# yahoo/bftkv

Measured on AMD Instinct MI355X. Metric: pgp_rsa2048_signature_verifies_per_sec, higher is better.
Workload: dtype u32; 1 GPU; 64-replica quorum, 10000 RSA-2048 signed writes per GPU (cfg2 of BASELINE.json), 534164 signature packets per GPU, 1.0% corrupt / 0.5% unknown issuer / 0.5% duplicate / 1.0% one-short; parallelism=shard-by-write x1, RCCL all-gather of verdict bitmaps on the verifier's stream, replicas=64, writes_per_gpu=10000, sigs_per_gpu=534164, batches_in_flight=3

## Files before the change

bftkv_amd/csrc/capi.hip:

```cpp
#include "../../include/bftkv_gpu.h"

#include <hip/hip_runtime.h>
#include <stdio.h>
#include <stdlib.h>
#include <string.h>

#include <limits.h>
#include <linux/futex.h>
#include <sched.h>
#include <sys/syscall.h>
#include <unistd.h>

#include <algorithm>
#include <array>
#include <atomic>
#include <memory>
#include <functional>
#include <map>
#include <set>
#include <chrono>
#include <condition_variable>
#include <mutex>
#include <shared_mutex>
#include <system_error>
// ... 33 lines not shown
  hipError_t ensure_exact(size_t bytes) {
    if (bytes <= cap) return hipSuccess;
    if (p) { hipError_t e = hipFree(p); if (e != hipSuccess) return e; p = nullptr; cap = 0; }
    hipError_t e = hipMalloc(&p, bytes);
    if (e == hipSuccess) cap = bytes;
    return e;
  }
  void release() { if (p) (void)hipFree(p); p = nullptr; cap = 0; }
  template <typename T> T* as() const { return (T*)p; }
};

struct KeyEntry {
  uint64_t key_id = 0, entity_id = 0;
  uint8_t algo = 0, flags = 0;
  uint32_t bits = 0, e = 0, n0 = 0, qbits = 0, n0_29 = 0;
  std::vector<uint32_t> nl29, r2_29;
  std::vector<uint32_t> nl, r2, r2w, qw, dtab, qpow, qconst;
  std::string material;
  bool cert_only = false;
  int cert_group = -1;
  uint32_t entity_index = 0;
  std::string cert_digest;
  uint64_t last_used = 0;
  bool dsa_unslotted = false;
};

struct QuorumHost {
  bool live = false;
  int n_qcs = 0;
  int32_t f[MAX_QC], mn[MAX_QC], thr[MAX_QC], suff[MAX_QC];
// ... 520 lines not shown
                           c->hash_mask.as<uint32_t>(), c->mid.as<uint32_t>(), c->mid64.as<uint64_t>());
        hipLaunchKernelGGL(k_hash_mid_text, dim3((n_items + 63) / 64, N_HASHES), dim3(64), 0, sh, d_tbs, d_tbs_off, n_items, c->hash_mask.as<uint32_t>(), txt);
      }
      hipLaunchKernelGGL(k_digest_sha256, dim3((total + 255) / 256), dim3(256), 0, sh, d_tbs, d_tbs_off, d_ss,
                         d_mid_in ? d_mid_in : c->mid.as<uint32_t>(), c->mid64.as<uint64_t>(), n_items, c->recs.as<SigRec>(), total,
                         c->digests.as<uint32_t>(), d_tbs_prefix, n_recs_dev);
    }
    HIPCHK(c, rec(6, sh));
    return 0;
  };
  if (!upload_tbs) { int hrc = hash_stream_work(); if (hrc) return hrc; }
  const dim3 qg((total + MODEXP_BLOCK / MONT_TPI - 1) / (MODEXP_BLOCK / MONT_TPI));
  const dim3 qg8((total + MODEXP_BLOCK / MONT_TPI_BIG - 1) / (MODEXP_BLOCK / MONT_TPI_BIG));
  static const bool wide8_off = getenv("BFTKV_NO_WIDE8") != nullptr;
  const bool wide8 = staged_cap != 0 && ss_len / 256 <= 8192 && !wide8_off;
  auto launch_modexp = [&](const uint32_t* start) {
    if (wide8)
      hipLaunchKernelGGL((k_rsa_modexp<10, MONT_TPI_BIG>), qg8, dim3(MODEXP_BLOCK), 0, s, d_ss, c->recs.as<SigRec>(), c->pk_list.as<uint32_t>(),
                         cnt_p, start, c->kt, c->r.as<uint32_t>(), c->xr.as<uint32_t>(), (uint64_t*)(cnt_p + 16));
    else {
#if BFTKV_RSA_FORM == 29
      hipLaunchKernelGGL((k_rsa_modexp<RSA29_L, MONT_TPI, RSA29_W>), qg, dim3(MODEXP_BLOCK), c->modexp_lds_pad, s, d_ss, c->recs.as<SigRec>(), c->pk_list.as<uint32_t>(),
                         cnt_p, start, c->kt, c->r.as<uint32_t>(), c->xr.as<uint32_t>(), (uint64_t*)(cnt_p + 16), (const uint32_t*)(cnt_p + 5));
      hipLaunchKernelGGL((k_rsa_modexp<MONT_L, MONT_TPI, MONT_W, true>), qg, dim3(MODEXP_BLOCK), c->modexp_lds_pad, s, d_ss, c->recs.as<SigRec>(), c->pk_list.as<uint32_t>(),
                         cnt_p, start, c->kt, c->r.as<uint32_t>(), c->xr.as<uint32_t>(), (uint64_t*)nullptr, (const uint32_t*)(cnt_p + 5));
#else
      hipLaunchKernelGGL((k_rsa_modexp<MONT_L, MONT_TPI>), qg, dim3(MODEXP_BLOCK), c->modexp_lds_pad, s, d_ss, c->recs.as<SigRec>(), c->pk_list.as<uint32_t>(),
                         cnt_p, start, c->kt, c->r.as<uint32_t>(), c->xr.as<uint32_t>(), (uint64_t*)(cnt_p + 16));
#endif
    }
    if (c->have_rsa3072)
      hipLaunchKernelGGL((k_rsa_modexp<MONT_L3072, MONT_TPI_BIG>), qg8, dim3(MODEXP_BLOCK), 0, s, d_ss, c->recs.as<SigRec>(), c->pk_list3072.as<uint32_t>(),
                         cnt_p + 2, start + 2, c->kt, c->r3072.as<uint32_t>(), c->xr.as<uint32_t>(), (uint64_t*)nullptr);
    if (c->have_rsa4096)
      hipLaunchKernelGGL((k_rsa_modexp<MONT_L4096, MONT_TPI_BIG>), qg8, dim3(MODEXP_BLOCK), 0, s, d_ss, c->recs.as<SigRec>(), c->pk_list4096.as<uint32_t>(),
                         cnt_p + 3, start + 3, c->kt, c->r4096.as<uint32_t>(), c->xr.as<uint32_t>(), (uint64_t*)nullptr);
  };
  static const bool turnstile_off = getenv("BFTKV_NO_TURNSTILE") != nullptr;
  const bool big = staged_cap ? (ev_input != nullptr && ss_len / 320 >= TURNSTILE_MIN_PACKETS) : total >= TURNSTILE_MIN_PACKETS;
  if (big && !turnstile_off) {
    Turnstile& g = g_turnstile[(unsigned)c->device & 15u];
    std::lock_guard<std::mutex> tl(g.mu);
    if (g.last && g.owner != c) HIPCHK(c, hipStreamWaitEvent(s, g.last, 0));
    HIPCHK(c, rec(9, s));
    launch_modexp(start0);
    if (!c->ev_turn) HIPCHK(c, hipEventCreateWithFlags(&c->ev_turn, hipEventDisableTiming));
    HIPCHK(c, hipEventRecord(c->ev_turn, s));
    g.last = c->ev_turn; g.owner = c;
  } else {
    HIPCHK(c, rec(9, s));
    if (total) launch_modexp(start0);
// ... 13 lines not shown
    for (uint32_t it = 0;; ++it) {
      const uint32_t v = __atomic_load_n(&c->h_mail[3], __ATOMIC_ACQUIRE);
      if (v) { other_hashes = (v & 1u) != 0; break; }
      if ((it & 255u) == 255u && std::chrono::steady_clock::now() - t_spin > std::chrono::microseconds(300) + std::chrono::nanoseconds((uint64_t)total / 2)) break;
      __builtin_ia32_pause();
    }
  }
  if (total && !d_mid_in && other_hashes)
    hipLaunchKernelGGL(k_digest_other, dim3(std::min<uint32_t>((total + 255) / 256, DIGEST_OTHER_MAX_BLOCKS)), dim3(256), 0, s,
                       d_tbs, d_tbs_off, d_ss, c->mid.as<uint32_t>(), c->mid64.as<uint64_t>(), n_items, c->recs.as<SigRec>(), total,
                       c->digests.as<uint32_t>(), c->pk_count.as<uint32_t>() + 4, txt, n_recs_dev);
  const dim3 cg(((uint64_t)total * CMP_LANES + 255) / 256);
  auto launch_compare = [&](const uint32_t* start) {
    hipLaunchKernelGGL(k_rsa_compare, cg, dim3(256), 0, s, c->recs.as<SigRec>(), c->pk_list.as<uint32_t>(),
                       cnt_p, start, c->kt, c->r.as<uint32_t>(), c->digests.as<uint32_t>());
    if (c->have_rsa3072)
      hipLaunchKernelGGL(k_rsa_compare, cg, dim3(256), 0, s, c->recs.as<SigRec>(), c->pk_list3072.as<uint32_t>(),
                         cnt_p + 2, start + 2, c->kt, c->r3072.as<uint32_t>(), c->digests.as<uint32_t>());
    if (c->have_rsa4096)
      hipLaunchKernelGGL(k_rsa_compare, cg, dim3(256), 0, s, c->recs.as<SigRec>(), c->pk_list4096.as<uint32_t>(),
                         cnt_p + 3, start + 3, c->kt, c->r4096.as<uint32_t>(), c->digests.as<uint32_t>());
  };
  auto launch_dsa = [&](const uint32_t* start) {
    hipLaunchKernelGGL(k_dsa_mul, dim3((total + 63) / 64), dim3(64), 0, s, c->recs.as<SigRec>(), c->dsa_list.as<uint32_t>(),
                       cnt_p, start, c->kt, c->digests.as<uint32_t>(), c->dsa_u.as<uint32_t>());
    const uint32_t* idx_s = nullptr; const uint32_t* idx_b = nullptr; const uint32_t* cnt_cls = nullptr;
    if (c->have_dsa3072 && c->have_dsa2048) {
      uint32_t* cc = cnt_p + (start == start0 ? 20 : 22);
      uint32_t* is = c->dsa_idx.as<uint32_t>() + (start == start0 ? 0 : 2 * (size_t)total);
      hipLaunchKernelGGL(k_dsa_split, dim3((total + 255) / 256), dim3(256), 0, s, c->recs.as<SigRec>(), c->dsa_list.as<uint32_t>(), cnt_p, start, c->kt,
// ... 44 lines not shown
  e.material.push_back((char)k.usable_sign);
  auto app = [&](const uint8_t* p, uint32_t l) {
    uint32_t z = 0;
    while (z < l && p[z] == 0) ++z;
    if (l > z) e.material.append((const char*)p + z, l - z);
    e.material.push_back('|');
  };
  app(k.n, k.n_len); app(k.e, k.e_len); app(k.g, k.g_len); app(k.y, k.y_len);
  e.flags = 0;
  if (k.usable_sign) e.flags |= KEYF_USABLE_SIGN;
  if (k.pk_algo != PK_RSA_ENCRYPT_ONLY && k.pk_algo != PK_ELGAMAL) e.flags |= KEYF_CAN_SIGN;
  if (k.key_id == k.entity_id) e.flags |= KEYF_PRIMARY;
  if (cert_only) e.flags |= KEYF_CERT_ONLY;
  e.bits = (uint32_t)hostbn::bit_length(k.n, k.n_len);
  e.e = 0; e.n0 = 0; e.qbits = 0;
  e.r2w.clear(); e.nl29.clear(); e.r2_29.clear(); e.n0_29 = 0;
  e.nl.assign(MONT_NMAX, 0); e.r2.assign(MONT_NMAX, 0); e.qw.assign(8, 0); e.dtab.assign(2 * DSA_N_BIG, 0); e.qpow.clear(); e.qconst.clear();
  if (k.pk_algo == PK_RSA || k.pk_algo == PK_RSA_SIGN_ONLY) {
    if (hostbn::bit_length(k.e, k.e_len) > 32) return fail(c, BFTKV_E_UNSUPPORTED, "RSA public exponent wider than 32 bits");
    for (uint32_t j = 0; j < k.e_len; ++j) e.e = (e.e << 8) | k.e[j];
    const int nlimbs = e.bits <= 2048 ? MONT_N : (e.bits <= 3072 ? MONT_TPI_BIG * MONT_L3072 : MONT_TPI_BIG * MONT_L4096);
    if (e.bits > 4096) e.bits = 0xFFFFFFFFu;
    else if (!hostbn::mont_setup(k.n, k.n_len, nlimbs, e.nl.data(), e.r2.data(), &e.n0)) e.bits = 0xFFFFFFFFu;
    else if (e.bits <= 2048) {
      std::vector<uint32_t> nl80(80);
      uint32_t n0b = 0;
      e.r2w.assign(80, 0);
      (void)hostbn::mont_setup(k.n, k.n_len, 80, nl80.data(), e.r2w.data(), &n0b);
      e.nl29.assign(RSA29_N, 0); e.r2_29.assign(RSA29_N, 0);
      (void)hostbn::mont_setup(k.n, k.n_len, RSA29_N, e.nl29.data(), e.r2_29.data(), &e.n0_29, RSA29_W);
    }
  } else if (k.pk_algo == PK_DSA) {
    e.qbits = (uint32_t)hostbn::bit_length(k.e, k.e_len);
    const int NLp = e.bits <= 2048 ? (int)DSA_N_SMALL : (int)DSA_N_BIG;
    const uint32_t cap_bits = e.bits <= 2048 ? 2048u : 3072u;
    const int nwords = (28 * NLp + 31) / 32 + 1;
    std::vector<uint32_t> p(nwords), g(nwords), y(nwords), q(nwords);
    hostbn::from_be(k.e, k.e_len, q.data(), nwords);
    bool ok = e.bits >= 2 && e.bits <= 3072 && e.qbits >= 32 && e.qbits <= 256 && (q[0] & 1u) &&
              hostbn::mont_setup(k.n, k.n_len, NLp, e.nl.data(), e.r2.data(), &e.n0);
    if (ok && (hostbn::bit_length(k.g, k.g_len) > cap_bits || hostbn::bit_length(k.y, k.y_len) > cap_bits)) ok = false;
    if (ok) {
      hostbn::from_be(k.n, k.n_len, p.data(), nwords);
      hostbn::from_be(k.g, k.g_len, g.data(), nwords);
      hostbn::from_be(k.y, k.y_len, y.data(), nwords);
// ... 187 lines not shown
                         (uint32_t)cs.size(), d_slots.as<uint32_t>(), d_rows.as<uint32_t>(), c->kt, c->dsa_comb.as<uint32_t>(), parts);
    else
      hipLaunchKernelGGL((k_dsa_build_comb<MONT_L, MONT_TPI>), dim3((n_groups + QUADS_PER_BLOCK - 1) / QUADS_PER_BLOCK), dim3(RSA_BLOCK), 0, c->stream,
                         (uint32_t)cs.size(), d_slots.as<uint32_t>(), d_rows.as<uint32_t>(), c->kt, c->dsa_comb.as<uint32_t>(), parts);
    e = hipStreamSynchronize(c->stream);
    d_slots.release(); d_rows.release();
  }
  if (e != hipSuccess) return fail(c, BFTKV_E_DEVICE, "k_dsa_build_comb", e);
  return 0;
}

int upload_key_table(bftkv_gpu_ctx* c) {
  if (c->root) return fail(c, BFTKV_E_STATE, "a forked context cannot change the key table (use its root)");
  KtWrite kw(c);
  std::vector<uint64_t> key_id, entity_ids;
  std::vector<uint32_t> entity, bits, e32, nl, r2, r2w, n0, qw, qbits, dtab, nl29, r2_29, n0_29;
  std::vector<uint8_t> algo, flags;
  auto add29 = [&](const KeyEntry& e) {
    nl29.insert(nl29.end(), e.nl29.begin(), e.nl29.end()); nl29.resize(key_id.size() * RSA29_N, 0);
    r2_29.insert(r2_29.end(), e.r2_29.begin(), e.r2_29.end()); r2_29.resize(key_id.size() * RSA29_N, 0);
    n0_29.push_back(e.n0_29);
  };
  std::vector<const KeyEntry*> rows;
  auto add = [&](const KeyEntry& e, bool own_entity) {
    uint32_t ent = 0;
    if (own_entity) { ent = (uint32_t)entity_ids.size(); entity_ids.push_back(e.entity_id); }
    else {
      for (; ent < entity_ids.size(); ++ent) if (entity_ids[ent] == e.entity_id) break;
      if (ent == entity_ids.size()) entity_ids.push_back(e.entity_id);
    }
    key_id.push_back(e.key_id); entity.push_back(ent); algo.push_back(e.algo); flags.push_back(e.flags);
    bits.push_back(e.bits); e32.push_back(e.e); n0.push_back(e.n0); qbits.push_back(e.qbits);
    nl.insert(nl.end(), e.nl.begin(), e.nl.end()); r2.insert(r2.end(), e.r2.begin(), e.r2.end());
    r2w.insert(r2w.end(), e.r2w.begin(), e.r2w.end()); r2w.resize(key_id.size() * 80, 0);
    add29(e);
    qw.insert(qw.end(), e.qw.begin(), e.qw.end()); dtab.insert(dtab.end(), e.dtab.begin(), e.dtab.end());
// ... 15 lines not shown
      add29(e);
      qw.insert(qw.end(), e.qw.begin(), e.qw.end()); dtab.insert(dtab.end(), e.dtab.begin(), e.dtab.end());
      rows.push_back(&e);
    }
    const_cast<KeyEntry&>(e).entity_index = group_ent;
    if (e.cert_group >= 0) {
      if (group_ents.size() <= (size_t)e.cert_group) group_ents.resize((size_t)e.cert_group + 1, 0xFFFFFFFEu);
      group_ents[(size_t)e.cert_group] = group_ent;
    }
  }
  std::vector<uint32_t> sorted_slot(key_id.size());
  for (size_t i = 0; i < sorted_slot.size(); ++i) sorted_slot[i] = (uint32_t)i;
  std::stable_sort(sorted_slot.begin(), sorted_slot.end(), [&](uint32_t a, uint32_t b) { return key_id[a] < key_id[b]; });
  std::vector<uint64_t> sorted_id(key_id.size());
  for (size_t i = 0; i < sorted_slot.size(); ++i) sorted_id[i] = key_id[sorted_slot[i]];
  int rc;
  if ((rc = upload(c, c->k_sorted_id, sorted_id)) || (rc = upload(c, c->k_sorted_slot, sorted_slot))) return rc;
  if ((rc = upload(c, c->k_id, key_id)) || (rc = upload(c, c->k_entity, entity)) || (rc = upload(c, c->k_algo, algo)) ||
      (rc = upload(c, c->k_flags, flags)) || (rc = upload(c, c->k_bits, bits)) || (rc = upload(c, c->k_e, e32)) ||
      (rc = upload(c, c->k_n, nl)) || (rc = upload(c, c->k_r2, r2)) || (rc = upload(c, c->k_n0, n0)) ||
      (rc = upload(c, c->k_q, qw)) || (rc = upload(c, c->k_qbits, qbits)) || (rc = upload(c, c->k_dsatab, dtab)) || (rc = upload(c, c->k_r2w, r2w)) ||
      (rc = upload(c, c->k_n29, nl29)) || (rc = upload(c, c->k_r2_29, r2_29)) || (rc = upload(c, c->k_n0_29, n0_29)))
    return rc;
  c->kt.r2_limbs80 = c->k_r2w.as<uint32_t>();
  c->kt.n_limbs29 = c->k_n29.as<uint32_t>(); c->kt.r2_limbs29 = c->k_r2_29.as<uint32_t>(); c->kt.n0inv29 = c->k_n0_29.as<uint32_t>();
  c->n_keys = (uint32_t)key_id.size();
  c->kt.n_keys = c->n_keys;
  c->kt.n_limbs = c->k_n.as<uint32_t>();
  c->kt.r2_limbs = c->k_r2.as<uint32_t>();
  c->kt.n0inv = c->k_n0.as<uint32_t>();
// ... 1124 lines not shown
```

bftkv_amd/csrc/device_types.h:

```cpp
#pragma once
#include <stdint.h>

namespace bftkv {

enum SigStatus : uint8_t {
  ST_OK = 0,
  ST_UNKNOWN_ISSUER = 1,
  ST_PARSE_ERROR = 2,
  ST_NOT_SIGNATURE = 3,
  ST_NO_ISSUER = 4,
  ST_HASH_UNSUPPORTED = 5,
  ST_HASH_TAG = 6,
  ST_ALGO_MISMATCH = 7,
  ST_BAD_SIG = 8,
  ST_KEY_CANNOT_SIGN = 9,
  ST_UNSUPPORTED = 10,
  ST_NOT_EXAMINED = 11,
  ST_PENDING_CHUNKED = 98,
  ST_PENDING_PARSE = 99,
  ST_PENDING_HASH = 100,
  ST_PENDING_RSA = 101,
  ST_PENDING_DSA = 102,
};

// ... 33 lines not shown
  const uint32_t* r2_limbs;
  const uint32_t* r2_limbs80;
  const uint32_t* n0inv;
  const uint32_t* n_limbs29;
  const uint32_t* r2_limbs29;
  const uint32_t* n0inv29;
  const uint32_t* q_words;
  const uint32_t* q_bits;
  const uint32_t* dsa_tab;
  const uint32_t* dsa_slot;
  const uint32_t* dsa_comb;
  uint32_t dsa_wbits;
  uint32_t dsa_entry_limbs;
  uint32_t hash_policy;
};
constexpr uint32_t dsa_nwin(uint32_t wbits) { return (256u + wbits - 1u) / wbits; }
constexpr uint32_t DSA_N_SMALL = 76, DSA_N_BIG = 112;
constexpr uint64_t dsa_comb_limbs_per_key(uint32_t wbits, uint32_t entry_limbs) {
  return 2ull * dsa_nwin(wbits) * ((1u << wbits) - 1u) * entry_limbs;
}
constexpr uint32_t dsa_qpow_words(uint32_t entry_limbs) { return entry_limbs * 10u; }
constexpr uint32_t dsa_qtail_words(uint32_t entry_limbs) { return dsa_qpow_words(entry_limbs) + 12u; }
constexpr bool dsa_plain_window(uint32_t base, uint32_t w, uint32_t nwin) { return base == 1u && w == nwin - 1u; }
constexpr uint64_t dsa_slot_stride(uint32_t wbits, uint32_t entry_limbs) { return dsa_comb_limbs_per_key(wbits, entry_limbs) + dsa_qtail_words(entry_limbs); }

constexpr uint8_t KEYF_USABLE_SIGN = 1, KEYF_CAN_SIGN = 2, KEYF_PRIMARY = 4;
constexpr uint8_t KEYF_CERT_ONLY = 8;
constexpr uint8_t KEYF_CERT_CHECK_ONLY = 16;
constexpr uint8_t KEYF_AMBIGUOUS = 32;
constexpr uint32_t ITEM_FENCED = 0x80000000u;
// ... 21 lines not shown
```

bftkv_amd/csrc/host_bignum.h:

```cpp
#pragma once
#include <stdint.h>
#include <string.h>

#include <vector>

namespace bftkv {
namespace hostbn {

constexpr int W28 = 28;
constexpr uint32_t MASK28 = (1u << W28) - 1;

inline void from_be(const uint8_t* be, uint32_t len, uint32_t* w, int nwords) {
  memset(w, 0, sizeof(uint32_t) * nwords);
  for (uint32_t i = 0; i < len; ++i) {
    uint32_t k = len - 1 - i;
    if ((int)(k >> 2) < nwords) w[k >> 2] |= (uint32_t)be[i] << (8 * (k & 3));
  }
}

inline int bit_length(const uint8_t* be, uint32_t len) {
  uint32_t i = 0;
  while (i < len && be[i] == 0) ++i;
  if (i == len) return 0;
  int top = 8;
// ... 122 lines not shown
  const uint32_t e = 2u * (uint32_t)W * (uint32_t)nlimbs;
  int hb = 31;
  while (!((e >> hb) & 1u)) --hb;
  for (int b = hb - 1; b >= 0; --b) {
    montmul64(acc.data(), acc.data(), m.data(), m0inv, k, acc.data());
    if ((e >> b) & 1u) dbl_mod64(acc.data(), m.data(), k);
  }
  one[0] = 1;
  montmul64(acc.data(), one.data(), m.data(), m0inv, k, acc.data());
  std::vector<uint32_t> r(nwords, 0);
  for (int i = 0; i < nwords && i < 2 * k; ++i) r[i] = (uint32_t)(acc[i >> 1] >> (32 * (i & 1)));
  to_limbs(r.data(), nwords, r2_limbs, nlimbs, W);
  return true;
}

inline void add_mod(uint32_t* a, const uint32_t* b, const uint32_t* m, int n) {
  uint64_t c = 0;
  for (int i = 0; i < n; ++i) { c += (uint64_t)a[i] + b[i]; a[i] = (uint32_t)c; c >>= 32; }
  if (c || cmp(a, m, n) >= 0) sub(a, m, n);
}
inline void mul_mod(const uint32_t* a, const uint32_t* b, const uint32_t* m, uint32_t* r, int n) {
  std::vector<uint32_t> acc(n, 0);
  for (int i = 32 * n - 1; i >= 0; --i) {
    dbl_mod(acc.data(), m, n);
    if ((b[i >> 5] >> (i & 31)) & 1u) add_mod(acc.data(), a, m, n);
  }
  memcpy(r, acc.data(), sizeof(uint32_t) * n);
}
inline void reduce(uint32_t* a, const uint32_t* m, int n) {
  std::vector<uint32_t> r(n, 0);
// ... 19 lines not shown
```

bftkv_amd/csrc/kernels.hip:

```cpp
#include <hip/hip_runtime.h>
#include <stdint.h>

#include "device_types.h"
#include "mont28.h"
#include "value_load.h"
#include "u256.h"
#include "hashes.h"

namespace bftkv {

struct ParsedPacket {
  uint64_t next;
  bool event;
  SigRec rec;
};

__host__ __device__ __forceinline__ bool known_tag(uint32_t tag) {
  return tag < 32 && ((0x00066BFEu >> tag) & 1u);
}

struct SubpacketState {
  bool have_ctime = false, have_issuer = false, have_embedded = false;
  bool too_deep = false;
  uint64_t issuer = 0;
// ... 1104 lines not shown
  }
  recs[ri].status = st;
}

constexpr int RSA_BLOCK = 256;
constexpr int QUADS_PER_BLOCK = RSA_BLOCK / MONT_TPI;
#ifndef BFTKV_MODEXP_BLOCK
#define BFTKV_MODEXP_BLOCK 256
#endif
constexpr int MODEXP_BLOCK = BFTKV_MODEXP_BLOCK;
#ifndef BFTKV_RSA_FORM
#define BFTKV_RSA_FORM 29
#endif
static_assert(BFTKV_RSA_FORM == 28 || BFTKV_RSA_FORM == 29, "BFTKV_RSA_FORM: 28 or 29");

enum : int { OP_TO_MONT = 0, OP_SQR = 1, OP_MULX = 2, OP_MULP = 3, OP_MUL1 = 4 };

constexpr int EM_LOW_BYTES = 84;
constexpr int EM_LOW_LIMBS = EM_LOW_BYTES * 8 / MONT_W;
static_assert(EM_LOW_LIMBS * MONT_W == EM_LOW_BYTES * 8, "the EM split must fall on a limb boundary");
constexpr uint32_t EM_HEAD_BAD = 0xFFFFFFFFu;

template <int W = MONT_W>
__device__ __forceinline__ uint32_t em_head_limb(uint32_t gi, uint32_t kbytes) {
  const int32_t top = 8 * ((int32_t)kbytes - 2), lo = (int32_t)gi * W;
  if (top < lo) return 0u;
  if (top >= lo + W - 1) return (1u << W) - 1u;
  return (1u << (top - lo + 1)) - 1u;
}

template <int L, int TPI, int W = MONT_W, bool WIDE_ONLY = false>
__global__ void __launch_bounds__(MODEXP_BLOCK, 3) k_rsa_modexp(const uint8_t* __restrict__ sig_blob, const SigRec* __restrict__ recs,
                                                          const uint32_t* __restrict__ pk_list, const uint32_t* __restrict__ pk_count_ptr,
                                                          const uint32_t* __restrict__ pk_start_ptr,
                                                          KeyTableDev kt, uint32_t* __restrict__ r_low,
                                                          uint32_t* __restrict__ xr_scratch, uint64_t* __restrict__ clk,
                                                          const uint32_t* __restrict__ wide_word = nullptr) {
  static_assert(W == MONT_W || (W == 29 && L == 18 && TPI == 4 && !WIDE_ONLY), "the only form at another radix is 18 x 4 at 2^29");
  constexpr int NL = TPI * L;
  constexpr int GROUPS = MODEXP_BLOCK / TPI;
  const bool stamp = clk && blockIdx.x == 0 && threadIdx.x == 0;
  uint64_t t0 = 0, r0 = 0;
  if (stamp) { t0 = __builtin_readcyclecounter(); r0 = __builtin_amdgcn_s_memrealtime(); }
  __shared__ uint32_t a_sh[GROUPS * NL];
  __shared__ uint32_t x_sh[GROUPS * NL];
  const uint32_t count = *pk_count_ptr, start = *pk_start_ptr;
  if (start + blockIdx.x * GROUPS >= count) return;
  if constexpr (WIDE_ONLY) { if (*wide_word == 0u) return; }
  const uint32_t quad = threadIdx.x / TPI;
  const int qlane = threadIdx.x % TPI;
  const uint32_t gq = start + blockIdx.x * GROUPS + quad;
  bool active = gq < count;
  if constexpr (W != MONT_W || WIDE_ONLY) {
    const bool wide = active && (recs[pk_list[gq]].flags & SIGF_WIDE_VALUE) != 0;
    active = active && (wide == WIDE_ONLY);
// ... 26 lines not shown
#pragma unroll
      for (int k = 0; k < L; ++k) x_lds[k] = x[k];
    } else {
      auto sig_b = [&](uint32_t i) -> uint32_t { return i < nb ? mp[nb - 1 - i] : 0u; };
#pragma unroll
      for (int k = 0; k < L; ++k) x_lds[k] = limb_of<W>(sig_b, qlane * L + k);
    }
  }
  const uint32_t n0inv = W == 29 ? kt.n0inv29[key] : kt.n0inv[key];
  const uint32_t e = kt.rsa_e[key];
  const uint32_t kbytes = (kt.mod_bits[key] + 7) >> 3;
  const uint32_t cls = (e << 1) | (((e & 1u) && e > 1u && !(rec.flags & 1u)) ? 1u : 0u);

  uint64_t todo = __builtin_amdgcn_ballot_w64(true);
  while (todo) {
    const int lead = __builtin_ctzll(todo);
    const uint32_t cls_u = (uint32_t)__builtin_amdgcn_readlane((int)cls, lead);
    const bool live = (cls == cls_u);
    const uint32_t e_u = cls_u >> 1;
    const bool sc_u = cls_u & 1u;
    const int top = 31 - __builtin_clz(e_u | 1u);
    int kind = OP_TO_MONT, bitpos = top;
    while (true) {
      if (kind == OP_TO_MONT) {
#pragma unroll
        for (int k = 0; k < L; ++k) { b[k] = rp[k]; a_lds[k] = x_lds[k]; }
      } else {
#pragma unroll
        for (int k = 0; k < L; ++k) b[k] = y[k];
        if (kind == OP_SQR) {
#pragma unroll
          for (int k = 0; k < L; ++k) a_lds[k] = y[k];
        } else if (kind == OP_MULX) {
#pragma unroll
          for (int k = 0; k < L; ++k) a_lds[k] = xrp[k];
        } else if (kind == OP_MULP) {
#pragma unroll
          for (int k = 0; k < L; ++k) a_lds[k] = x_lds[k];
        } else {
#pragma unroll
          for (int k = 0; k < L; ++k) a_lds[k] = (qlane == 0 && k == 0) ? 1u : 0u;
        }
      }
      __builtin_amdgcn_fence(__ATOMIC_ACQ_REL, "wavefront");
      if (kind == OP_SQR) mont_mul<L, TPI, true, W>(y, a_rd, b, n, n0inv, qlane);
      else mont_mul<L, TPI, false, W>(y, a_rd, b, n, n0inv, qlane);
      __builtin_amdgcn_fence(__ATOMIC_ACQ_REL, "wavefront");
      if (kind == OP_TO_MONT && (e_u & (e_u - 1u)) != 0 && !(sc_u && __builtin_popcount(e_u) == 2)) {
#pragma unroll
        for (int k = 0; k < L; ++k) xrp[k] = y[k];
      }
      if (kind == OP_MULP || kind == OP_MUL1) break;
      if (kind == OP_SQR && ((e_u >> bitpos) & 1u)) { kind = (bitpos == 0 && sc_u) ? OP_MULP : OP_MULX; continue; }
      --bitpos;
      kind = (bitpos >= 0) ? OP_SQR : OP_MUL1;
    }
    canonicalize<L, TPI, W>(y, qlane);
    if (e_u == 0) {
#pragma unroll
      for (int k = 0; k < L; ++k) y[k] = (qlane == 0 && k == 0) ? 1u : 0u;
    }
    uint32_t head = 0;
    if constexpr (W == MONT_W) {
#pragma unroll
      for (int k = 0; k < L; ++k) {
        const uint32_t gi = (uint32_t)qlane * L + k;
        if (gi >= (uint32_t)EM_LOW_LIMBS) head |= y[k] ^ em_head_limb(gi, kbytes);
      }
    } else {
#pragma unroll
      for (int k = 0; k < L; ++k) {
        const int32_t lo = ((int32_t)qlane * L + k) * W, cut = 8 * EM_LOW_BYTES;
// ... 97 lines not shown
  {
    const uint32_t n_valid = min((uint32_t)GROUPS, count - q0) * EM_LOW_LIMBS;
    const uint32_t* src = r_low + (uint64_t)q0 * EM_LOW_LIMBS;
    for (uint32_t t = threadIdx.x; t < GROUPS * EM_LOW_LIMBS; t += 256) r_sh[t] = t < n_valid ? src[t] : 0u;
    __syncthreads();
  }
  const uint32_t* rp = r_sh + (threadIdx.x / CMP_LANES) * EM_LOW_LIMBS + qlane * CMP_L;
  uint32_t diff = 0;
#pragma unroll
  for (int k = 0; k < CMP_L; ++k) {
    const int bit = MONT_W * k, wi = bit >> 5, sh = bit & 31;
    const uint32_t em = (sh == 0 ? Wn[wi] : __builtin_amdgcn_alignbit(Wn[wi + 1], Wn[wi], sh)) & MONT_MASK;
    diff |= em ^ rp[k];
  }
  diff = quad_or(diff);
  if (active && pending && qlane == 0) recs[ri].status = (diff == 0) ? ST_OK : ST_BAD_SIG;
}

constexpr int DSA_U_WORDS = 24;
__device__ __forceinline__ const uint32_t* dsa_slot_base(const KeyTableDev& kt, uint32_t key) {
  return kt.dsa_comb + (uint64_t)kt.dsa_slot[key] * dsa_slot_stride(kt.dsa_wbits, kt.dsa_entry_limbs);
}
__device__ __forceinline__ const uint32_t* dsa_qconst(const KeyTableDev& kt, uint32_t key) {
  return dsa_slot_base(kt, key) + dsa_comb_limbs_per_key(kt.dsa_wbits, kt.dsa_entry_limbs) + dsa_qpow_words(kt.dsa_entry_limbs);
}
__global__ void __launch_bounds__(64) k_dsa_inv(const uint8_t* __restrict__ sig_blob, const SigRec* __restrict__ recs,
                                                const uint32_t* __restrict__ dsa_list, const uint32_t* __restrict__ pk_count,
                                                const uint32_t* __restrict__ pk_start,
                                                KeyTableDev kt, uint32_t* __restrict__ dsa_u , uint32_t batch_min) {
  if (pk_count[1] - pk_start[1] >= batch_min) return;
  const uint32_t di = pk_start[1] + blockIdx.x * blockDim.x + threadIdx.x;
// ... 741 lines not shown
```

bftkv_amd/csrc/mont28.h:

```cpp
#pragma once
#include <hip/hip_runtime.h>
#include <stdint.h>

namespace bftkv {

constexpr int MONT_W = 28;
constexpr uint32_t MONT_MASK = (1u << MONT_W) - 1;
constexpr int MONT_TPI = 4;
constexpr int MONT_L = 19;
constexpr int MONT_N = MONT_TPI * MONT_L;
constexpr int MONT_TPI_BIG = 8;
constexpr int MONT_L3072 = 14, MONT_L4096 = 19;
constexpr int MONT_NMAX = MONT_TPI_BIG * MONT_L4096;

constexpr int DPP_QUAD_BCAST0 = 0x00;
constexpr int DPP_QUAD_SHR1 = 0x90;
constexpr int DPP_QUAD_SWAP1 = 0xB1;
constexpr int DPP_QUAD_SWAP2 = 0x4E;
constexpr int DPP_ROW_SHL1 = 0x101;

__device__ __forceinline__ uint32_t dpp_quad_bcast0(uint32_t v) {
  return (uint32_t)__builtin_amdgcn_update_dpp(0, (int)v, DPP_QUAD_BCAST0, 0xF, 0xF, true);
}
__device__ __forceinline__ uint32_t dpp_quad_shr1(uint32_t v) {
// ... 50 lines not shown
    if (r > 0) in = dpp_row_shl1((uint32_t)Q[(O + r - 1) % M]) & mask_v;
#pragma unroll
    for (int k = SQR ? r : 0; k < L; ++k) {
      const uint32_t av = (SQR && k > r) ? ai2 : ai;
      if (k == L - 1 && r > 0) Q[(O + r + k) % M] = mad64(av, b[k], in);
      else Q[(O + r + k) % M] = mad64(av, b[k], Q[(O + r + k) % M]);
    }
    const uint32_t m = grp_bcast0<TPI>((uint32_t)Q[(O + r) % M] * n0inv, qlane) & mask_v;
#pragma unroll
    for (int k = 0; k < L; ++k) Q[(O + r + k) % M] = mad64(m, n[k], Q[(O + r + k) % M]);
    Q[(O + r + 1) % M] += Q[(O + r) % M] >> W;
  }
  Q[(O + M - 1) % M] = dpp_row_shl1((uint32_t)Q[(O + L - 1) % M]) & mask_v;
}

template <int L, int TPI = MONT_TPI, bool SQR = false, int W = MONT_W>
__device__ __forceinline__ void mont_mul(uint32_t (&out)[L], const uint32_t* a_lds,
                                         const uint32_t (&b)[L], const uint32_t (&n)[L],
                                         uint32_t n0inv, int qlane) {
  constexpr bool NORM = 2 * TPI * L > 255;
  static_assert(TPI % 2 == 0, "the ring window runs two blocks per loop iteration");
  static_assert(W == 28 || (W == 29 && !NORM && L <= 18), "a 29-bit limb fits the column only in a ring form of at most 18 rows per block");
  constexpr uint32_t MASK = (1u << W) - 1;
  uint32_t mask_v;
  if constexpr (W == 28) asm("v_mov_b32 %0, 0xfffffff" : "=v"(mask_v));
  else asm("v_mov_b32 %0, 0x1fffffff" : "=v"(mask_v));
  uint64_t Q[NORM ? 2 * L - 1 : 2 * L];
#pragma unroll
  for (int k = 0; k < L + (NORM ? 1 : 0); ++k) Q[k] = 0;

  if constexpr (!NORM) {
#pragma unroll 1
    for (int blk = 0; blk < TPI; blk += 2) {
      mont_block_ring<L, TPI, SQR, 0, W>(Q, a_lds + blk * L, b, n, n0inv, qlane, mask_v);
      mont_block_ring<L, TPI, SQR, L, W>(Q, a_lds + (blk + 1) * L, b, n, n0inv, qlane, mask_v);
    }
  } else {
#pragma unroll 1
    for (int blk = 0; blk < TPI; ++blk) {
      const uint32_t* ap = a_lds + blk * L;
#pragma unroll
      for (int r = 0; r < L; ++r) {
        const uint32_t ai = ap[r];
        const uint32_t ai2 = ai << 1;
#pragma unroll
        for (int k = SQR ? r : 0; k < L; ++k) {
// ... 8 lines not shown
      }
#pragma unroll
      for (int k = 0; k < L; ++k) {
        const uint64_t nx = dpp_row_shl1((uint32_t)Q[k]) & mask_v;
        Q[k] = (k < L - 1) ? Q[L + k] + nx : nx;
      }
#pragma unroll
      for (int k = 0; k < L; ++k) {
        const uint64_t c = Q[k] >> W;
        Q[k] &= MASK;
        if (k < L - 1) Q[k + 1] += c; else Q[L] = c;
      }
    }
  }

  uint64_t c = 0;
#pragma unroll
  for (int k = 0; k < L; ++k) {
    uint64_t v = Q[k] + c;
    out[k] = (uint32_t)v & MASK;
    c = v >> W;
  }
  if (NORM) c += Q[L];
  uint32_t clo = grp_shr1<TPI>((uint32_t)c), chi = grp_shr1<TPI>((uint32_t)(c >> 32));
  uint64_t cin = (qlane == 0) ? 0 : (((uint64_t)chi << 32) | clo);
  uint64_t v0 = (uint64_t)out[0] + cin;
  out[0] = (uint32_t)v0 & MASK;
  uint32_t v1 = out[1] + (uint32_t)(v0 >> W);
  out[1] = v1 & MASK;
  out[2] += v1 >> W;
}

template <int L, int TPI = MONT_TPI, int W = MONT_W>
__device__ __forceinline__ void canonicalize(uint32_t (&x)[L], int qlane) {
// ... 49 lines not shown
```

Baseline: 167.6 million verifies/s.

## Verify RSA by comparing s^(e-1) against precomputed expected-message Montgomery products

Adds a default-on plain ladder for 29-bit RSA. The modexp stops one multiply early, computing s^(e-1) in plain form via a leading squaring that skips the to-Montgomery conversion, and writes it to scratch with a full-row marker. A new compare kernel builds the digest tail, multiplies it by per-key precomputed tables (EM*acc constants and per-hash padding heads) using a reduced-block Montgomery product, adds the head term, and checks equality. This drops the final multiply and conversion from the ladder, at the cost of extra host table setup, more key-table memory and an extra compare launch.

```diff
diff --git a/bftkv_amd/csrc/capi.hip b/bftkv_amd/csrc/capi.hip
--- a/bftkv_amd/csrc/capi.hip
+++ b/bftkv_amd/csrc/capi.hip
@@ -71,6 +71,7 @@
   uint64_t key_id = 0, entity_id = 0;
   uint8_t algo = 0, flags = 0;
   uint32_t bits = 0, e = 0, n0 = 0, qbits = 0, n0_29 = 0;
+  std::vector<uint32_t> em29;
   std::vector<uint32_t> nl29, r2_29;
   std::vector<uint32_t> nl, r2, r2w, qw, dtab, qpow, qconst;
   std::string material;
@@ -621,7 +622,25 @@
   const dim3 qg8((total + MODEXP_BLOCK / MONT_TPI_BIG - 1) / (MODEXP_BLOCK / MONT_TPI_BIG));
   static const bool wide8_off = getenv("BFTKV_NO_WIDE8") != nullptr;
   const bool wide8 = staged_cap != 0 && ss_len / 256 <= 8192 && !wide8_off;
+  auto launch_modexp_big = [&](const uint32_t* start) {
+    if (c->have_rsa3072)
+      hipLaunchKernelGGL((k_rsa_modexp<MONT_L3072, MONT_TPI_BIG>), qg8, dim3(MODEXP_BLOCK), 0, s, d_ss, c->recs.as<SigRec>(), c->pk_list3072.as<uint32_t>(),
+                         cnt_p + 2, start + 2, c->kt, c->r3072.as<uint32_t>(), c->xr.as<uint32_t>(), (uint64_t*)nullptr);
+    if (c->have_rsa4096)
+      hipLaunchKernelGGL((k_rsa_modexp<MONT_L4096, MONT_TPI_BIG>), qg8, dim3(MODEXP_BLOCK), 0, s, d_ss, c->recs.as<SigRec>(), c->pk_list4096.as<uint32_t>(),
+                         cnt_p + 3, start + 3, c->kt, c->r4096.as<uint32_t>(), c->xr.as<uint32_t>(), (uint64_t*)nullptr);
+  };
   auto launch_modexp = [&](const uint32_t* start) {
+#if BFTKV_RSA_FORM == 29 && BFTKV_RSA_PLAIN_LADDER
+    if (!wide8) {
+      launch_modexp_big(start);
+      hipLaunchKernelGGL((k_rsa_modexp<MONT_L, MONT_TPI, MONT_W, true>), qg, dim3(MODEXP_BLOCK), c->modexp_lds_pad, s, d_ss, c->recs.as<SigRec>(), c->pk_list.as<uint32_t>(),
+                         cnt_p, start, c->kt, c->r.as<uint32_t>(), c->xr.as<uint32_t>(), (uint64_t*)nullptr, (const uint32_t*)(cnt_p + 5));
+      hipLaunchKernelGGL((k_rsa_modexp<RSA29_L, MONT_TPI, RSA29_W>), qg, dim3(MODEXP_BLOCK), c->modexp_lds_pad, s, d_ss, c->recs.as<SigRec>(), c->pk_list.as<uint32_t>(),
+                         cnt_p, start, c->kt, c->r.as<uint32_t>(), c->xr.as<uint32_t>(), (uint64_t*)(cnt_p + 16), (const uint32_t*)(cnt_p + 5));
+      return;
+    }
+#endif
     if (wide8)
       hipLaunchKernelGGL((k_rsa_modexp<10, MONT_TPI_BIG>), qg8, dim3(MODEXP_BLOCK), 0, s, d_ss, c->recs.as<SigRec>(), c->pk_list.as<uint32_t>(),
                          cnt_p, start, c->kt, c->r.as<uint32_t>(), c->xr.as<uint32_t>(), (uint64_t*)(cnt_p + 16));
@@ -636,12 +655,7 @@
                          cnt_p, start, c->kt, c->r.as<uint32_t>(), c->xr.as<uint32_t>(), (uint64_t*)(cnt_p + 16));
 #endif
     }
-    if (c->have_rsa3072)
-      hipLaunchKernelGGL((k_rsa_modexp<MONT_L3072, MONT_TPI_BIG>), qg8, dim3(MODEXP_BLOCK), 0, s, d_ss, c->recs.as<SigRec>(), c->pk_list3072.as<uint32_t>(),
-                         cnt_p + 2, start + 2, c->kt, c->r3072.as<uint32_t>(), c->xr.as<uint32_t>(), (uint64_t*)nullptr);
-    if (c->have_rsa4096)
-      hipLaunchKernelGGL((k_rsa_modexp<MONT_L4096, MONT_TPI_BIG>), qg8, dim3(MODEXP_BLOCK), 0, s, d_ss, c->recs.as<SigRec>(), c->pk_list4096.as<uint32_t>(),
-                         cnt_p + 3, start + 3, c->kt, c->r4096.as<uint32_t>(), c->xr.as<uint32_t>(), (uint64_t*)nullptr);
+    launch_modexp_big(start);
   };
   static const bool turnstile_off = getenv("BFTKV_NO_TURNSTILE") != nullptr;
   const bool big = staged_cap ? (ev_input != nullptr && ss_len / 320 >= TURNSTILE_MIN_PACKETS) : total >= TURNSTILE_MIN_PACKETS;
@@ -685,6 +699,11 @@
   auto launch_compare = [&](const uint32_t* start) {
     hipLaunchKernelGGL(k_rsa_compare, cg, dim3(256), 0, s, c->recs.as<SigRec>(), c->pk_list.as<uint32_t>(),
                        cnt_p, start, c->kt, c->r.as<uint32_t>(), c->digests.as<uint32_t>());
+#if BFTKV_RSA_FORM == 29 && BFTKV_RSA_PLAIN_LADDER
+    if (!wide8)
+      hipLaunchKernelGGL(k_rsa_compare_full, cg, dim3(256), 0, s, c->recs.as<SigRec>(), c->pk_list.as<uint32_t>(),
+                         cnt_p, start, c->kt, c->r.as<uint32_t>(), c->xr.as<uint32_t>(), c->digests.as<uint32_t>());
+#endif
     if (c->have_rsa3072)
       hipLaunchKernelGGL(k_rsa_compare, cg, dim3(256), 0, s, c->recs.as<SigRec>(), c->pk_list3072.as<uint32_t>(),
                          cnt_p + 2, start + 2, c->kt, c->r3072.as<uint32_t>(), c->digests.as<uint32_t>());
@@ -759,7 +778,7 @@
   if (cert_only) e.flags |= KEYF_CERT_ONLY;
   e.bits = (uint32_t)hostbn::bit_length(k.n, k.n_len);
   e.e = 0; e.n0 = 0; e.qbits = 0;
-  e.r2w.clear(); e.nl29.clear(); e.r2_29.clear(); e.n0_29 = 0;
+  e.r2w.clear(); e.nl29.clear(); e.r2_29.clear(); e.n0_29 = 0; e.em29.clear();
   e.nl.assign(MONT_NMAX, 0); e.r2.assign(MONT_NMAX, 0); e.qw.assign(8, 0); e.dtab.assign(2 * DSA_N_BIG, 0); e.qpow.clear(); e.qconst.clear();
   if (k.pk_algo == PK_RSA || k.pk_algo == PK_RSA_SIGN_ONLY) {
     if (hostbn::bit_length(k.e, k.e_len) > 32) return fail(c, BFTKV_E_UNSUPPORTED, "RSA public exponent wider than 32 bits");
@@ -774,6 +793,12 @@
       (void)hostbn::mont_setup(k.n, k.n_len, 80, nl80.data(), e.r2w.data(), &n0b);
       e.nl29.assign(RSA29_N, 0); e.r2_29.assign(RSA29_N, 0);
       (void)hostbn::mont_setup(k.n, k.n_len, RSA29_N, e.nl29.data(), e.r2_29.data(), &e.n0_29, RSA29_W);
+#if BFTKV_RSA_PLAIN_LADDER
+      if ((e.e & 1u) && e.e > 1u) {
+        e.em29.assign(EM29_ROWS * EM29_LIMBS, 0);
+        (void)hostbn::em_tables(k.n, k.n_len, e.e, RSA29_N, RSA29_W, RSA29_L, EM29_TL, N_HASHES, e.em29.data(), e.em29.data() + EM29_ROW_HEAD * EM29_LIMBS);
+      }
+#endif
     }
   } else if (k.pk_algo == PK_DSA) {
     e.qbits = (uint32_t)hostbn::bit_length(k.e, k.e_len);
@@ -991,12 +1016,15 @@
   if (c->root) return fail(c, BFTKV_E_STATE, "a forked context cannot change the key table (use its root)");
   KtWrite kw(c);
   std::vector<uint64_t> key_id, entity_ids;
-  std::vector<uint32_t> entity, bits, e32, nl, r2, r2w, n0, qw, qbits, dtab, nl29, r2_29, n0_29;
+  std::vector<uint32_t> entity, bits, e32, nl, r2, r2w, n0, qw, qbits, dtab, nl29, r2_29, n0_29, em29;
   std::vector<uint8_t> algo, flags;
   auto add29 = [&](const KeyEntry& e) {
     nl29.insert(nl29.end(), e.nl29.begin(), e.nl29.end()); nl29.resize(key_id.size() * RSA29_N, 0);
     r2_29.insert(r2_29.end(), e.r2_29.begin(), e.r2_29.end()); r2_29.resize(key_id.size() * RSA29_N, 0);
     n0_29.push_back(e.n0_29);
+#if BFTKV_RSA_PLAIN_LADDER
+    em29.insert(em29.end(), e.em29.begin(), e.em29.end()); em29.resize(key_id.size() * EM29_ROWS * EM29_LIMBS, 0);
+#endif
   };
   std::vector<const KeyEntry*> rows;
   auto add = [&](const KeyEntry& e, bool own_entity) {
@@ -1042,6 +1070,7 @@
   std::stable_sort(sorted_slot.begin(), sorted_slot.end(), [&](uint32_t a, uint32_t b) { return key_id[a] < key_id[b]; });
   std::vector<uint64_t> sorted_id(key_id.size());
   for (size_t i = 0; i < sorted_slot.size(); ++i) sorted_id[i] = key_id[sorted_slot[i]];
+  r2_29.insert(r2_29.end(), em29.begin(), em29.end());
   int rc;
   if ((rc = upload(c, c->k_sorted_id, sorted_id)) || (rc = upload(c, c->k_sorted_slot, sorted_slot))) return rc;
   if ((rc = upload(c, c->k_id, key_id)) || (rc = upload(c, c->k_entity, entity)) || (rc = upload(c, c->k_algo, algo)) ||
diff --git a/bftkv_amd/csrc/device_types.h b/bftkv_amd/csrc/device_types.h
--- a/bftkv_amd/csrc/device_types.h
+++ b/bftkv_amd/csrc/device_types.h
@@ -1,5 +1,14 @@
 #pragma once
 #include <stdint.h>
+
+#define BFTKV_RSA_LADDER_mont 0
+#define BFTKV_RSA_LADDER_plain 1
+#ifndef BFTKV_RSA_LADDER
+#define BFTKV_RSA_LADDER plain
+#endif
+#define BFTKV_LADDER_CAT_(a, b) a##b
+#define BFTKV_LADDER_CAT(a, b) BFTKV_LADDER_CAT_(a, b)
+#define BFTKV_RSA_PLAIN_LADDER BFTKV_LADDER_CAT(BFTKV_RSA_LADDER_, BFTKV_RSA_LADDER)
 
 namespace bftkv {
 
@@ -71,6 +80,13 @@
   uint32_t dsa_entry_limbs;
   uint32_t hash_policy;
 };
+constexpr uint32_t EM29_ROWS = 9, EM29_LIMBS = 72, EM29_ROW_HEAD = 2;
+constexpr uint32_t EM29_TL[7] = {51, 47, 35, 83, 67, 34, 34};
+#ifdef __HIPCC__
+__device__ __forceinline__ const uint32_t* em29_rows(const KeyTableDev& kt, uint32_t key) {
+  return kt.r2_limbs29 + (uint64_t)kt.n_keys * EM29_LIMBS + (uint64_t)key * (EM29_ROWS * EM29_LIMBS);
+}
+#endif
 constexpr uint32_t dsa_nwin(uint32_t wbits) { return (256u + wbits - 1u) / wbits; }
 constexpr uint32_t DSA_N_SMALL = 76, DSA_N_BIG = 112;
 constexpr uint64_t dsa_comb_limbs_per_key(uint32_t wbits, uint32_t entry_limbs) {
diff --git a/bftkv_amd/csrc/host_bignum.h b/bftkv_amd/csrc/host_bignum.h
--- a/bftkv_amd/csrc/host_bignum.h
+++ b/bftkv_amd/csrc/host_bignum.h
@@ -160,6 +160,61 @@
   return true;
 }
 
+inline void half_mod64(uint64_t* a, const uint64_t* m, int k) {
+  unsigned __int128 c = 0;
+  if (a[0] & 1ull) for (int i = 0; i < k; ++i) { c += (unsigned __int128)a[i] + m[i]; a[i] = (uint64_t)c; c >>= 64; }
+  for (int i = 0; i < k; ++i) a[i] = (a[i] >> 1) | (i + 1 < k ? a[i + 1] << 63 : 0ull);
+}
+
+inline bool em_tables(const uint8_t* n_be, uint32_t n_len, uint32_t e, int nlimbs, int W, int block, const uint32_t* tl, int n_hashes,
+                      uint32_t* emc, uint32_t* emh) {
+  memset(emc, 0, sizeof(uint32_t) * 2 * (size_t)nlimbs);
+  memset(emh, 0, sizeof(uint32_t) * (size_t)n_hashes * (size_t)nlimbs);
+  const int nwords = (W * nlimbs + 31) / 32 + 1;
+  std::vector<uint32_t> n(nwords);
+  from_be(n_be, n_len, n.data(), nwords);
+  const int bits = bit_length(n_be, n_len);
+  if ((n[0] & 1) == 0 || bits < 2 || bits > W * nlimbs - 2 || (e & 1u) == 0 || e < 3) return false;
+  const int k = (bits + 64) / 64;
+  std::vector<uint64_t> m(k, 0), one(k, 0), rinv(k, 0), acc(k, 0), t(k, 0), plain1(k, 0);
+  for (int i = 0; i < nwords && i < 2 * k; ++i) m[i >> 1] |= (uint64_t)n[i] << (32 * (i & 1));
+  uint64_t m0inv = m[0];
+  for (int i = 0; i < 6; ++i) m0inv *= 2ull - m[0] * m0inv;
+  m0inv = 0ull - m0inv;
+  one[(bits - 1) >> 6] = 1ull << ((bits - 1) & 63);
+  for (int i = bits - 1; i < 64 * k; ++i) dbl_mod64(one.data(), m.data(), k);
+  rinv = one;
+  for (int i = 0; i < W * nlimbs; ++i) half_mod64(rinv.data(), m.data(), k);
+  acc = one;
+  const uint32_t d = e - 1u;
+  for (int b = 31; b >= 0; --b) {
+    montmul64(acc.data(), acc.data(), m.data(), m0inv, k, acc.data());
+    if ((d >> b) & 1u) montmul64(acc.data(), rinv.data(), m.data(), m0inv, k, acc.data());
+  }
+  plain1[0] = 1;
+  auto put = [&](const uint64_t* v, uint32_t* limbs) {
+    std::vector<uint32_t> r(nwords, 0);
+    for (int i = 0; i < nwords && i < 2 * k; ++i) r[i] = (uint32_t)(v[i >> 1] >> (32 * (i & 1)));
+    to_limbs(r.data(), nwords, limbs, nlimbs, W);
+  };
+  t = acc;
+  for (int j = 0; j < 2; ++j) {
+    for (int i = 0; i < W * block; ++i) dbl_mod64(t.data(), m.data(), k);
+    std::vector<uint64_t> o(k);
+    montmul64(t.data(), plain1.data(), m.data(), m0inv, k, o.data());
+    put(o.data(), emc + (size_t)j * nlimbs);
+  }
+  const uint32_t kb = ((uint32_t)bits + 7u) >> 3;
+  for (int h = 0; h < n_hashes; ++h) {
+    if (kb < tl[h] + 11u) continue;
+    std::vector<uint64_t> head(k, 0), o(k);
+    for (uint32_t bit = 8u * tl[h] + 8u; bit < 8u * kb - 15u; ++bit) head[bit >> 6] |= 1ull << (bit & 63u);
+    montmul64(head.data(), acc.data(), m.data(), m0inv, k, o.data());
+    put(o.data(), emh + (size_t)h * nlimbs);
+  }
+  return true;
+}
+
 inline void add_mod(uint32_t* a, const uint32_t* b, const uint32_t* m, int n) {
   uint64_t c = 0;
   for (int i = 0; i < n; ++i) { c += (uint64_t)a[i] + b[i]; a[i] = (uint32_t)c; c >>= 32; }
diff --git a/bftkv_amd/csrc/kernels.hip b/bftkv_amd/csrc/kernels.hip
--- a/bftkv_amd/csrc/kernels.hip
+++ b/bftkv_amd/csrc/kernels.hip
@@ -1142,12 +1142,13 @@
 #endif
 static_assert(BFTKV_RSA_FORM == 28 || BFTKV_RSA_FORM == 29, "BFTKV_RSA_FORM: 28 or 29");
 
-enum : int { OP_TO_MONT = 0, OP_SQR = 1, OP_MULX = 2, OP_MULP = 3, OP_MUL1 = 4 };
+enum : int { OP_TO_MONT = 0, OP_SQR = 1, OP_MULX = 2, OP_MULP = 3, OP_MUL1 = 4, OP_SQRX = 5 };
 
 constexpr int EM_LOW_BYTES = 84;
 constexpr int EM_LOW_LIMBS = EM_LOW_BYTES * 8 / MONT_W;
 static_assert(EM_LOW_LIMBS * MONT_W == EM_LOW_BYTES * 8, "the EM split must fall on a limb boundary");
 constexpr uint32_t EM_HEAD_BAD = 0xFFFFFFFFu;
+constexpr uint32_t EM_FULL_ROW = 0xFFFFFFFEu;
 
 template <int W = MONT_W>
 __device__ __forceinline__ uint32_t em_head_limb(uint32_t gi, uint32_t kbytes) {
@@ -1167,6 +1168,7 @@
   static_assert(W == MONT_W || (W == 29 && L == 18 && TPI == 4 && !WIDE_ONLY), "the only form at another radix is 18 x 4 at 2^29");
   constexpr int NL = TPI * L;
   constexpr int GROUPS = MODEXP_BLOCK / TPI;
+  constexpr bool PLAIN = W == 29 && BFTKV_RSA_PLAIN_LADDER != 0;
   const bool stamp = clk && blockIdx.x == 0 && threadIdx.x == 0;
   uint64_t t0 = 0, r0 = 0;
   if (stamp) { t0 = __builtin_readcyclecounter(); r0 = __builtin_amdgcn_s_memrealtime(); }
@@ -1223,17 +1225,31 @@
 
   uint64_t todo = __builtin_amdgcn_ballot_w64(true);
   while (todo) {
-    const int lead = __builtin_ctzll(todo);
+    const uint64_t first = PLAIN ? (todo & __builtin_amdgcn_ballot_w64((cls & 1u) == 0u)) : 0ull;
+    const int lead = __builtin_ctzll(first ? first : todo);
     const uint32_t cls_u = (uint32_t)__builtin_amdgcn_readlane((int)cls, lead);
     const bool live = (cls == cls_u);
     const uint32_t e_u = cls_u >> 1;
     const bool sc_u = cls_u & 1u;
     const int top = 31 - __builtin_clz(e_u | 1u);
     int kind = OP_TO_MONT, bitpos = top;
+    const bool plain_u = PLAIN && sc_u;
+    if constexpr (PLAIN) {
+      if (plain_u) {
+        kind = OP_SQRX; bitpos = top - 1;
+        if (__builtin_popcount(e_u) > 2 && live) {
+#pragma unroll
+          for (int k = 0; k < L; ++k) xrp[k] = x_lds[k];
+        }
+      }
+    }
     while (true) {
       if (kind == OP_TO_MONT) {
 #pragma unroll
         for (int k = 0; k < L; ++k) { b[k] = rp[k]; a_lds[k] = x_lds[k]; }
+      } else if (PLAIN && kind == OP_SQRX) {
+#pragma unroll
+        for (int k = 0; k < L; ++k) { b[k] = x_lds[k]; a_lds[k] = b[k]; }
       } else {
 #pragma unroll
         for (int k = 0; k < L; ++k) b[k] = y[k];
@@ -1252,7 +1268,8 @@
         }
       }
       __builtin_amdgcn_fence(__ATOMIC_ACQ_REL, "wavefront");
-      if (kind == OP_SQR) mont_mul<L, TPI, true, W>(y, a_rd, b, n, n0inv, qlane);
+      const bool sqr = kind == OP_SQR || (PLAIN && kind == OP_SQRX);
+      if (sqr) mont_mul<L, TPI, true, W>(y, a_rd, b, n, n0inv, qlane);
       else mont_mul<L, TPI, false, W>(y, a_rd, b, n, n0inv, qlane);
       __builtin_amdgcn_fence(__ATOMIC_ACQ_REL, "wavefront");
       if (kind == OP_TO_MONT && (e_u & (e_u - 1u)) != 0 && !(sc_u && __builtin_popcount(e_u) == 2)) {
@@ -1260,11 +1277,21 @@
         for (int k = 0; k < L; ++k) xrp[k] = y[k];
       }
       if (kind == OP_MULP || kind == OP_MUL1) break;
-      if (kind == OP_SQR && ((e_u >> bitpos) & 1u)) { kind = (bitpos == 0 && sc_u) ? OP_MULP : OP_MULX; continue; }
+      if (sqr && ((e_u >> bitpos) & 1u)) { kind = (bitpos == 0 && sc_u) ? OP_MULP : OP_MULX; continue; }
       --bitpos;
       kind = (bitpos >= 0) ? OP_SQR : OP_MUL1;
     }
     canonicalize<L, TPI, W>(y, qlane);
+    if (PLAIN && plain_u) {
+      reduce_once<L, TPI, W>(y, n, qlane);
+      if (live && active) {
+#pragma unroll
+        for (int k = 0; k < L; ++k) xrp[k] = y[k];
+        if (qlane == 0) r_low[(uint64_t)pi * EM_LOW_LIMBS] = EM_FULL_ROW;
+      }
+      todo &= ~__builtin_amdgcn_ballot_w64(live);
+      continue;
+    }
     if (e_u == 0) {
 #pragma unroll
       for (int k = 0; k < L; ++k) y[k] = (qlane == 0 && k == 0) ? 1u : 0u;
@@ -1392,7 +1419,86 @@
     diff |= em ^ rp[k];
   }
   diff = quad_or(diff);
+#if BFTKV_RSA_PLAIN_LADDER
+  if (r_sh[(threadIdx.x / CMP_LANES) * EM_LOW_LIMBS] == EM_FULL_ROW) return;
+#endif
   if (active && pending && qlane == 0) recs[ri].status = (diff == 0) ? ST_OK : ST_BAD_SIG;
+}
+
+__global__ void __launch_bounds__(256) k_rsa_compare_full(SigRec* __restrict__ recs, const uint32_t* __restrict__ pk_list,
+                                                          const uint32_t* __restrict__ pk_count_ptr, const uint32_t* __restrict__ pk_start_ptr,
+                                                          KeyTableDev kt, const uint32_t* __restrict__ r_low,
+                                                          const uint32_t* __restrict__ xr_scratch, const uint32_t* __restrict__ digests) {
+  constexpr int L = RSA29_L, TPI = MONT_TPI, W = RSA29_W, NL = RSA29_N;
+  constexpr int GROUPS = 256 / TPI;
+  constexpr int T_WORDS = 24;
+  constexpr int T_LIMBS = 2 * L;
+  const uint32_t count = *pk_count_ptr, start = *pk_start_ptr;
+  const uint32_t q0 = start + blockIdx.x * GROUPS;
+  if (q0 >= count) return;
+  const uint32_t grp = threadIdx.x / TPI;
+  const int qlane = threadIdx.x % TPI;
+  const uint32_t gq = q0 + grp;
+  const bool active = gq < count;
+  const uint32_t pi = active ? gq : (count - 1);
+  const bool full = r_low[(uint64_t)pi * EM_LOW_LIMBS] == EM_FULL_ROW;
+  if (!__any(active && full)) return;
+  const uint32_t ri = pk_list[pi];
+  const SigRec rec = recs[ri];
+  const bool mine = active && full && rec.status == ST_PENDING_RSA;
+  const uint32_t key = (uint32_t)rec.key_slot;
+  const HashInfo hi = hash_info(rec.hash_id);
+  const uint32_t hlen = hi.dlen, plen = hi.plen, tl = hlen + plen;
+  __shared__ uint32_t tw_sh[GROUPS * T_WORDS];
+  __shared__ uint32_t t_sh[GROUPS * T_LIMBS];
+  uint32_t* tw = tw_sh + grp * T_WORDS;
+  uint32_t* tlimbs = t_sh + grp * T_LIMBS;
+  const uint32_t* dgw = digests + (uint64_t)ri * 16;
+  const uint32_t hw = hlen >> 2;
+#pragma unroll
+  for (int t = 0; t < T_WORDS / TPI; ++t) {
+    const uint32_t w = (uint32_t)qlane * (T_WORDS / TPI) + t;
+    uint32_t v = 0;
+    if (w < hw) v = __builtin_bswap32(dgw[hw - 1 - w]);
+    else {
+#pragma unroll
+      for (uint32_t bq = 0; bq < 4; ++bq) {
+        const uint32_t i = 4 * w + bq;
+        if (i >= hlen && i < tl) v |= digestinfo_byte(rec.hash_id, plen - 1 - (i - hlen)) << (8 * bq);
+      }
+    }
+    tw[w] = v;
+  }
+  __builtin_amdgcn_fence(__ATOMIC_ACQ_REL, "wavefront");
+#pragma unroll
+  for (int t = 0; t < T_LIMBS / TPI; ++t) {
+    const uint32_t j = (uint32_t)qlane * (T_LIMBS / TPI) + t, bit = (uint32_t)W * j, wi = bit >> 5, sh = bit & 31u;
+    const uint64_t lo = wi < (uint32_t)T_WORDS ? tw[wi] : 0u, up = wi + 1 < (uint32_t)T_WORDS ? tw[wi + 1] : 0u;
+    tlimbs[j] = (uint32_t)(((up << 32) | lo) >> sh) & ((1u << W) - 1u);
+  }
+  __builtin_amdgcn_fence(__ATOMIC_ACQ_REL, "wavefront");
+  const bool two = __any(mine && tl > (uint32_t)(L * W / 8));
+  const uint32_t* em = em29_rows(kt, key);
+  const uint32_t* cp = em + (two ? 1u : 0u) * EM29_LIMBS + qlane * L;
+  const uint32_t* hp = em + (EM29_ROW_HEAD + (uint32_t)hi.idx) * EM29_LIMBS + qlane * L;
+  const uint32_t* np = kt.n_limbs29 + (uint64_t)key * NL + qlane * L;
+  const uint32_t n0inv = kt.n0inv29[key];
+  uint32_t n[L], b[L], y[L];
+#pragma unroll
+  for (int k = 0; k < L; ++k) { n[k] = np[k]; b[k] = cp[k]; }
+  if (two) mont_mul<L, TPI, false, W, 2>(y, tlimbs, b, n, n0inv, qlane);
+  else mont_mul<L, TPI, false, W, 1>(y, tlimbs, b, n, n0inv, qlane);
+#pragma unroll
+  for (int k = 0; k < L; ++k) y[k] += hp[k];
+  canonicalize<L, TPI, W>(y, qlane);
+  reduce_once<L, TPI, W>(y, n, qlane);
+  reduce_once<L, TPI, W>(y, n, qlane);
+  const uint32_t* zp = xr_scratch + (uint64_t)pi * NL + qlane * L;
+  uint32_t diff = 0;
+#pragma unroll
+  for (int k = 0; k < L; ++k) diff |= y[k] ^ zp[k];
+  diff = quad_or(diff);
+  if (mine && qlane == 0) recs[ri].status = (diff == 0) ? ST_OK : ST_BAD_SIG;
 }
 
 constexpr int DSA_U_WORDS = 24;
diff --git a/bftkv_amd/csrc/mont28.h b/bftkv_amd/csrc/mont28.h
--- a/bftkv_amd/csrc/mont28.h
+++ b/bftkv_amd/csrc/mont28.h
@@ -88,13 +88,14 @@
   Q[(O + M - 1) % M] = dpp_row_shl1((uint32_t)Q[(O + L - 1) % M]) & mask_v;
 }
 
-template <int L, int TPI = MONT_TPI, bool SQR = false, int W = MONT_W>
+template <int L, int TPI = MONT_TPI, bool SQR = false, int W = MONT_W, int NB = TPI>
 __device__ __forceinline__ void mont_mul(uint32_t (&out)[L], const uint32_t* a_lds,
                                          const uint32_t (&b)[L], const uint32_t (&n)[L],
                                          uint32_t n0inv, int qlane) {
   constexpr bool NORM = 2 * TPI * L > 255;
   static_assert(TPI % 2 == 0, "the ring window runs two blocks per loop iteration");
   static_assert(W == 28 || (W == 29 && !NORM && L <= 18), "a 29-bit limb fits the column only in a ring form of at most 18 rows per block");
+  static_assert(NB == TPI || (!NORM && !SQR && NB >= 1 && NB < TPI), "fewer blocks: general products on the ring only");
   constexpr uint32_t MASK = (1u << W) - 1;
   uint32_t mask_v;
   if constexpr (W == 28) asm("v_mov_b32 %0, 0xfffffff" : "=v"(mask_v));
@@ -103,7 +104,14 @@
 #pragma unroll
   for (int k = 0; k < L + (NORM ? 1 : 0); ++k) Q[k] = 0;
 
-  if constexpr (!NORM) {
+  if constexpr (!NORM && NB != TPI) {
+#pragma unroll 1
+    for (int blk = 0; blk + 1 < NB; blk += 2) {
+      mont_block_ring<L, TPI, SQR, 0, W>(Q, a_lds + blk * L, b, n, n0inv, qlane, mask_v);
+      mont_block_ring<L, TPI, SQR, L, W>(Q, a_lds + (blk + 1) * L, b, n, n0inv, qlane, mask_v);
+    }
+    if constexpr (NB % 2 != 0) mont_block_ring<L, TPI, SQR, 0, W>(Q, a_lds + (NB - 1) * L, b, n, n0inv, qlane, mask_v);
+  } else if constexpr (!NORM) {
 #pragma unroll 1
     for (int blk = 0; blk < TPI; blk += 2) {
       mont_block_ring<L, TPI, SQR, 0, W>(Q, a_lds + blk * L, b, n, n0inv, qlane, mask_v);
@@ -142,10 +150,11 @@
     }
   }
 
+  constexpr int RO = (NB % 2 != 0) ? L : 0;
   uint64_t c = 0;
 #pragma unroll
   for (int k = 0; k < L; ++k) {
-    uint64_t v = Q[k] + c;
+    uint64_t v = Q[RO + k] + c;
     out[k] = (uint32_t)v & MASK;
     c = v >> W;
   }
```

Measured after the change: 163.5 million verifies/s. 2.4% lower.
